# miha-stopar/Plonky3-mobile

Measured on AMD Instinct MI355X. Metric: fib_air proofs/sec, higher is better.
Workload: dtype u32 (BabyBear Montgomery, 31-bit modular)

## Files before the change

### plonky3-mobile_amd/csrc/mmcs.hip

```cpp
#include <algorithm>

#include "common.h"
#include "mmcs.h"
#include "poseidon2.hip.h"
#include "poseidon2_coop.hip.h"
#include "poseidon2_f64.hip.h"
#include "poseidon2_q4.hip.h"
#include "keccak.hip.h"

namespace p3 {

constexpr int MAX_CLASS_MATS = 16;

struct RowSet {
    const uint32_t* ptr[MAX_CLASS_MATS];
    uint32_t width[MAX_CLASS_MATS];
    uint32_t stride[MAX_CLASS_MATS];
    uint32_t count;
    uint32_t total;
};

__device__ __forceinline__ void load_digest(const uint32_t* p, uint32_t* out8) {
    const uint4* q = reinterpret_cast<const uint4*>(p);
    uint4 a = q[0], b = q[1];
    out8[0] = a.x; out8[1] = a.y; out8[2] = a.z; out8[3] = a.w;
    out8[4] = b.x; out8[5] = b.y; out8[6] = b.z; out8[7] = b.w;
}
__device__ __forceinline__ void store_digest(uint32_t* p, const uint32_t* s) {
    uint4* q = reinterpret_cast<uint4*>(p);
    q[0] = make_uint4(s[0], s[1], s[2], s[3]);
    q[1] = make_uint4(s[4], s[5], s[6], s[7]);
}

__device__ __forceinline__ void sponge_row(const RowSet& rs, uint64_t r, uint32_t (&s)[16]) {
#pragma unroll
    for (int i = 0; i < 16; i++) s[i] = 0;
    if (rs.count == 1) {
        const uint32_t* row = rs.ptr[0] + r * rs.stride[0];
        const uint32_t w = rs.width[0];
        for (uint32_t k = 0; k < w; k += 8) {
#pragma unroll
            for (int i = 0; i < 8; i++)
                if (k + i < w) s[i] = row[k + i];
            p2::permute(s);
        }
        return;
    }
    uint32_t m = 0, off = 0;
    for (uint32_t k = 0; k < rs.total; k += 8) {
#pragma unroll
        for (int i = 0; i < 8; i++) {
            if (k + i < rs.total) {
                while (off >= rs.width[m]) { m++; off = 0; }
                s[i] = rs.ptr[m][r * rs.stride[m] + off];
                off++;
            }
        }
        p2::permute(s);
    }
// ... 26 lines not shown
    }
    store_digest(next + i * 8, s);
}

__global__ void __launch_bounds__(256) tree_top_kernel(uint32_t* layer0, uint32_t n0) {
    P3_LATENCY_BOUND_KERNEL();
    extern __shared__ __attribute__((aligned(16))) uint32_t lds[];
    const uint32_t tid = threadIdx.x;
    for (uint32_t i = tid; i < n0 * 8; i += blockDim.x) lds[i] = layer0[i];
    __syncthreads();
    uint32_t* out = layer0 + (size_t)n0 * 8;
    for (uint32_t n = n0; n > 1; n >>= 1) {
        uint32_t half = n >> 1;
        uint32_t s[16];
        bool act = tid < half;
        if (act) {
#pragma unroll
            for (int k = 0; k < 16; k++) s[k] = lds[tid * 16 + k];
            p2::permute(s);
        }
        __syncthreads();
        if (act) {
#pragma unroll
            for (int k = 0; k < 8; k++) lds[tid * 8 + k] = s[k];
            store_digest(out + tid * 8, s);
        }
        __syncthreads();
        out += (size_t)half * 8;
    }
}


__global__ void __launch_bounds__(256) leaf_hash_f64_kernel(const uint32_t* mat, uint32_t width, uint64_t n_rows, uint32_t* digests) {
    if (gridDim.x <= 512u) P3_LATENCY_BOUND_KERNEL();
    uint64_t r = (uint64_t)blockIdx.x * blockDim.x + threadIdx.x;
    if (r >= n_rows) return;
    double s[16];
#pragma unroll
    for (int i = 0; i < 16; i++) s[i] = 0.0;
    const uint32_t* row = mat + r * width;
    for (uint32_t k = 0; k < width; k += 8) {
#pragma unroll
        for (int i = 0; i < 8; i++)
            if (k + i < width) s[i] = p2f::load_elem(row[k + i]);
        p2f::permute(s);
        if (k + 8 < width) {
#pragma unroll
            for (int i = 0; i < 16; i++) s[i] = p2f::reduce(s[i]);
        }
    }
    uint32_t d[8];
    const p2f::MagicRegs smk = p2f::magic_regs();
#pragma unroll
    for (int i = 0; i < 8; i++) d[i] = p2f::store_elem(s[i], smk);
    store_digest(digests + r * 8, d);
}
__global__ void __launch_bounds__(256) compress_layer_q4_kernel(const uint32_t* prev, uint32_t* next, uint64_t n_out, uint32_t prio) {
    if (prio) P3_LATENCY_BOUND_KERNEL();
    const uint32_t q = threadIdx.x & 3u;
    const uint64_t i = ((uint64_t)blockIdx.x * blockDim.x + threadIdx.x) >> 2;
    const bool act = i < n_out;
    const p2q::LaneConsts lc = p2q::lane_consts(q);
    double s[4] = {0.0, 0.0, 0.0, 0.0};
    if (act) {
        const uint4 w = *reinterpret_cast<const uint4*>(prev + i * 16 + 4 * q);
        s[0] = p2f::load_elem(w.x); s[1] = p2f::load_elem(w.y); s[2] = p2f::load_elem(w.z); s[3] = p2f::load_elem(w.w);
    }
    p2q::permute(s, lc, q == 0);
    if (act && q < 2) {
        const p2f::MagicRegs smk = p2f::magic_regs();
        *reinterpret_cast<uint4*>(next + i * 8 + 4 * q) =
            make_uint4(p2f::store_elem(s[0], smk), p2f::store_elem(s[1], smk), p2f::store_elem(s[2], smk), p2f::store_elem(s[3], smk));
    }
}
__global__ void __launch_bounds__(256) leaf_hash_q4_kernel(const uint32_t* mat, uint32_t width, uint64_t n_rows, uint32_t* digests, uint32_t prio) {
    if (prio) P3_LATENCY_BOUND_KERNEL();
    const uint32_t q = threadIdx.x & 3u;
    const uint64_t r = ((uint64_t)blockIdx.x * blockDim.x + threadIdx.x) >> 2;
    const bool act = r < n_rows;
    const p2q::LaneConsts lc = p2q::lane_consts(q);
    double s[4] = {0.0, 0.0, 0.0, 0.0};
    const uint32_t* row = mat + (act ? r : 0) * width;
    for (uint32_t k = 0; k < width; k += 8) {
        if (act && q < 2) {
#pragma unroll
            for (uint32_t i = 0; i < 4; i++)
                if (k + 4 * q + i < width) s[i] = p2f::load_elem(row[k + 4 * q + i]);
        }
        p2q::permute(s, lc, q == 0);
        if (k + 8 < width) {
#pragma unroll
            for (int i = 0; i < 4; i++) s[i] = p2f::reduce(s[i]);
        }
    }
    if (act && q < 2) {
        const p2f::MagicRegs smk = p2f::magic_regs();
        *reinterpret_cast<uint4*>(digests + r * 8 + 4 * q) =
            make_uint4(p2f::store_elem(s[0], smk), p2f::store_elem(s[1], smk), p2f::store_elem(s[2], smk), p2f::store_elem(s[3], smk));
    }
}
constexpr uint32_t LEAF_WIDE_CHUNK = 32, LEAF_WIDE_STRIDE = 36;
__global__ void __launch_bounds__(256) leaf_hash_f64_wide_kernel(const uint32_t* mat, uint32_t width, uint64_t n_rows, uint32_t* digests) {
    __shared__ __attribute__((aligned(16))) uint32_t tile[256 * LEAF_WIDE_STRIDE];
    const uint32_t tid = threadIdx.x, col = tid & 31u, rsub = tid >> 5;
    const uint64_t r0 = (uint64_t)blockIdx.x * 256u, r = r0 + tid;
    double s[16];
#pragma unroll
// ... 11 lines not shown
        __syncthreads();
#pragma unroll
        for (uint32_t i = 0; i < 32; i++) tile[(rsub + 8u * i) * LEAF_WIDE_STRIDE + col] = pre[i];
        __syncthreads();
        if (c0 + LEAF_WIDE_CHUNK < width) fetch(c0 + LEAF_WIDE_CHUNK);
        const uint4* mine = reinterpret_cast<const uint4*>(tile + tid * LEAF_WIDE_STRIDE);
#pragma unroll 1
        for (uint32_t k = 0; k < LEAF_WIDE_CHUNK && c0 + k < width; k += 8) {
            const uint4 a = mine[k / 4], b = mine[k / 4 + 1];
            const uint32_t w[8] = {a.x, a.y, a.z, a.w, b.x, b.y, b.z, b.w};
#pragma unroll
            for (int i = 0; i < 8; i++)
                if (c0 + k + i < width) s[i] = p2f::load_elem(w[i]);
            p2f::permute(s);
            if (c0 + k + 8 < width) {
#pragma unroll
                for (int i = 0; i < 16; i++) s[i] = p2f::reduce(s[i]);
            }
        }
    }
    if (r >= n_rows) return;
    uint32_t d[8];
    const p2f::MagicRegs smk = p2f::magic_regs();
#pragma unroll
    for (int i = 0; i < 8; i++) d[i] = p2f::store_elem(s[i], smk);
    store_digest(digests + r * 8, d);
}
__global__ void __launch_bounds__(256) leaf_hash_f64_rowset_kernel(RowSet rs, uint64_t n_rows, uint32_t* digests) {
    if (gridDim.x <= 512u) P3_LATENCY_BOUND_KERNEL();
    uint64_t r = (uint64_t)blockIdx.x * blockDim.x + threadIdx.x;
    if (r >= n_rows) return;
    double s[16];
#pragma unroll
    for (int i = 0; i < 16; i++) s[i] = 0.0;
    uint32_t m = 0, off = 0;
    for (uint32_t k = 0; k < rs.total; k += 8) {
#pragma unroll
        for (int i = 0; i < 8; i++) {
            if (k + i < rs.total) {
                while (off >= rs.width[m]) { m++; off = 0; }
                s[i] = p2f::load_elem(rs.ptr[m][r * rs.stride[m] + off]);
                off++;
            }
        }
        p2f::permute(s);
        if (k + 8 < rs.total) {
#pragma unroll
            for (int i = 0; i < 16; i++) s[i] = p2f::reduce(s[i]);
        }
    }
    uint32_t d[8];
    const p2f::MagicRegs smk = p2f::magic_regs();
#pragma unroll
    for (int i = 0; i < 8; i++) d[i] = p2f::store_elem(s[i], smk);
    store_digest(digests + r * 8, d);
}
__global__ void __launch_bounds__(256, 8) compress_layer_f64_kernel(const uint32_t* prev, uint32_t* next, uint64_t n_out) {
    if (gridDim.x <= 512u) P3_LATENCY_BOUND_KERNEL();
    uint64_t i = (uint64_t)blockIdx.x * blockDim.x + threadIdx.x;
    if (i >= n_out) return;
    uint32_t w[16];
    load_digest(prev + i * 16, w);
    load_digest(prev + i * 16 + 8, w + 8);
    double s[16];
#pragma unroll
    for (int k = 0; k < 16; k++) s[k] = p2f::load_elem(w[k]);
    p2f::permute(s);
    uint32_t d[8];
    const p2f::MagicRegs smk = p2f::magic_regs();
#pragma unroll
    for (int k = 0; k < 8; k++) d[k] = p2f::store_elem(s[k], smk);
    store_digest(next + i * 8, d);
}

__global__ void __launch_bounds__(256) compress_coop_kernel(const uint32_t* prev, uint32_t* next, uint32_t n_out) {
    P3_LATENCY_BOUND_KERNEL();
    const uint32_t lane16 = threadIdx.x & 15;
    const p2c::LaneConst lc = p2c::lane_constants(lane16);
    uint32_t i = (blockIdx.x * blockDim.x + threadIdx.x) >> 4;
    bool act = i < n_out;
    uint32_t v = act ? prev[(size_t)i * 16 + lane16] : 0u;
    v = p2c::permute(v, lc);
    if (act && lane16 < 8) next[(size_t)i * 8 + lane16] = v;
}
__global__ void __launch_bounds__(256) leaf_coop_kernel(const uint32_t* mat, uint32_t width, uint32_t n_rows, uint32_t* digests) {
    P3_LATENCY_BOUND_KERNEL();
    const uint32_t lane16 = threadIdx.x & 15;
    const p2c::LaneConst lc = p2c::lane_constants(lane16);
    uint32_t r = (blockIdx.x * blockDim.x + threadIdx.x) >> 4;
    bool act = r < n_rows;
    uint32_t v = 0;
    for (uint32_t k = 0; k < width; k += 8) {
        if (act && lane16 < 8 && k + lane16 < width) v = mat[(size_t)r * width + k + lane16];
        v = p2c::permute(v, lc);
    }
    if (act && lane16 < 8) digests[(size_t)r * 8 + lane16] = v;
}
__global__ void __launch_bounds__(1024) tree_levels_coop_kernel(uint32_t* layer_in, uint32_t n_in, uint32_t chunk, uint32_t levels,
                                                                uint32_t* root_copy) {
    P3_LATENCY_BOUND_KERNEL();
    __shared__ uint32_t lds[128 * 8];
    const uint32_t tid = threadIdx.x, lane16 = tid & 15, grp = tid >> 4;
    const p2c::LaneConst lc = p2c::lane_constants(lane16);
    const uint32_t* src = layer_in + (size_t)blockIdx.x * chunk * 8;
    for (uint32_t i = tid; i < chunk * 8; i += blockDim.x) lds[i] = src[i];
    __syncthreads();
    uint32_t* out = layer_in + (size_t)n_in * 8;
// ... 571 lines not shown
    constexpr uint32_t Q4_PRIO = 1;
    const uint64_t KCOOP_IN = profile == PROFILE_LATENCY ? (1ull << 12) : (1ull << 10);
    constexpr uint32_t KCOOP_CHUNK_LOG = 4;
    constexpr uint64_t KLANE_CHUNK = 1ull << 7;
    if (kind == HASH_KECCAK) {
        RowSet rs0 = make_rowset(*t, maxh);
        if (rs0.count == 1 && rs0.width[0] >= 68 && rs0.stride[0] == rs0.width[0])
            hipLaunchKernelGGL(keccak_leaf_wide_kernel, dim3((uint32_t)((maxh + 255) / 256)), dim3(256), 0, stream, rs0.ptr[0], rs0.width[0], maxh,
                               t->layers);
        else if (!launch_keccak_leaf_salted(stream, rs0, maxh, t->layers))
            hipLaunchKernelGGL(keccak_leaf_kernel, dim3((uint32_t)((maxh + 255) / 256)), dim3(256), 0, stream, rs0, maxh, t->layers);
        P3_HIP(hipGetLastError());
        for (size_t l = 1; l < t->layer_len.size(); l++) {
            uint64_t len = t->layer_len[l];
            RowSet rs = make_rowset(*t, len);
            if (len < COOP_MAX && !rs.count) {
                const uint64_t n_in = t->layer_len[l - 1];
                const bool coop = n_in <= KCOOP_IN;
                uint32_t levels = 0;
                while (levels < (coop ? KCOOP_CHUNK_LOG : 11u) && l + levels < t->layer_len.size() && !has_height(*t, t->layer_len[l + levels])) levels++;
                if (!coop) while (levels > 1 && (n_in >> levels) < KCOOP_IN) levels--;
                const uint32_t chunk = (uint32_t)std::min<uint64_t>(n_in, coop ? 1ull << KCOOP_CHUNK_LOG : KLANE_CHUNK);
                while ((1u << levels) > chunk) levels--;
                if (coop)
                    hipLaunchKernelGGL(keccak_tree_levels_coop_kernel, dim3((uint32_t)(n_in / chunk)), dim3(std::max<uint32_t>(64, chunk * 32)), 0,
                                       stream, t->layers + t->layer_off[l - 1], (uint32_t)n_in, chunk, levels, root_copy);
                else
                    hipLaunchKernelGGL(keccak_tree_levels_kernel, dim3((uint32_t)(n_in / chunk)), dim3(std::max<uint32_t>(64, chunk / 2)),
                                       (size_t)chunk * 32, stream, t->layers + t->layer_off[l - 1], (uint32_t)n_in, chunk, levels, root_copy);
                P3_HIP(hipGetLastError());
                if (t->layer_len[l + levels - 1] == 1) t->root_copied = root_copy != nullptr;
                l += levels - 1;
                continue;
            }
            hipLaunchKernelGGL(keccak_compress_kernel, dim3((uint32_t)((len + 255) / 256)), dim3(256), 0, stream,
                               t->layers + t->layer_off[l - 1], t->layers + t->layer_off[l], len, rs, rs.count > 0 ? 1u : 0u);
            P3_HIP(hipGetLastError());
        }
        *out = t.release();
        return OK;
    }
    {
        RowSet rs = make_rowset(*t, maxh);
        const bool dense1 = rs.count == 1 && rs.stride[0] == rs.width[0];
        if (dense1 && maxh < COOP_MAX && maxh * 16 <= 0x7fffffffull) {
            hipLaunchKernelGGL(leaf_coop_kernel, dim3((uint32_t)((maxh * 16 + 255) / 256)), dim3(256), 0, stream, rs.ptr[0],
                               rs.width[0], (uint32_t)maxh, t->layers);
        } else if (dense1 && maxh <= Q4_MAX && rs.width[0] <= 64 && (reinterpret_cast<uintptr_t>(t->layers) & 15u) == 0) {
            hipLaunchKernelGGL(leaf_hash_q4_kernel, dim3((uint32_t)((maxh * 4 + 255) / 256)), dim3(256), 0, stream, rs.ptr[0], rs.width[0], maxh,
                               t->layers, Q4_PRIO);
        } else if (dense1 && rs.width[0] >= 64) {
            hipLaunchKernelGGL(leaf_hash_f64_wide_kernel, dim3((uint32_t)((maxh + 255) / 256)), dim3(256), 0, stream, rs.ptr[0],
                               rs.width[0], maxh, t->layers);
        } else if (dense1) {
            hipLaunchKernelGGL(leaf_hash_f64_kernel, dim3((uint32_t)((maxh + 255) / 256)), dim3(256), 0, stream, rs.ptr[0],
                               rs.width[0], maxh, t->layers);
        } else if ((maxh >= COOP_MAX || (rs.count == 1 && !dense1))) {
            hipLaunchKernelGGL(leaf_hash_f64_rowset_kernel, dim3((uint32_t)((maxh + 255) / 256)), dim3(256), 0, stream, rs, maxh, t->layers);
        } else {
            hipLaunchKernelGGL(leaf_hash_kernel, dim3((uint32_t)((maxh + 255) / 256)), dim3(256), 0, stream, rs, maxh, t->layers);
        }
        P3_HIP(hipGetLastError());
    }
    for (size_t l = 1; l < t->layer_len.size();) {
        uint64_t len = t->layer_len[l];
        RowSet rs = make_rowset(*t, len);
        bool inject = rs.count > 0;
        if (!inject && len < COOP_MAX) {
            uint32_t levels = 0;
            while (levels < COOP_CHUNK_LOG && l + levels < t->layer_len.size() && !has_height(*t, t->layer_len[l + levels])) levels++;
            uint64_t n_in = t->layer_len[l - 1];
            uint32_t chunk = (uint32_t)std::min<uint64_t>(n_in, 1ull << COOP_CHUNK_LOG);
            while ((1u << levels) > chunk) levels--;
            uint32_t blocks = (uint32_t)(n_in / chunk);
            uint32_t threads = std::max<uint32_t>(64, chunk * 8);
            bool makes_root = t->layer_len[l + levels - 1] == 1;
            hipLaunchKernelGGL(tree_levels_coop_kernel, dim3(blocks), dim3(threads), 0, stream, t->layers + t->layer_off[l - 1],
                               (uint32_t)n_in, chunk, levels, makes_root ? root_copy : nullptr);
            P3_HIP(hipGetLastError());
            if (makes_root) t->root_copied = root_copy != nullptr;
            l += levels;
            continue;
        }
        if (!inject && len <= Q4_MAX) {
            hipLaunchKernelGGL(compress_layer_q4_kernel, dim3((uint32_t)((len * 4 + 255) / 256)), dim3(256), 0, stream,
                               t->layers + t->layer_off[l - 1], t->layers + t->layer_off[l], len, Q4_PRIO);
        } else if (!inject) {
            hipLaunchKernelGGL(compress_layer_f64_kernel, dim3((uint32_t)((len + 255) / 256)), dim3(256), 0, stream,
                               t->layers + t->layer_off[l - 1], t->layers + t->layer_off[l], len);
        } else {
            hipLaunchKernelGGL(compress_layer_kernel, dim3((uint32_t)((len + 255) / 256)), dim3(256), 0, stream,
                               t->layers + t->layer_off[l - 1], t->layers + t->layer_off[l], len, rs, inject ? 1u : 0u);
        }
        P3_HIP(hipGetLastError());
        l++;
    }
    *out = t.release();
    return OK;
}

int mmcs_root(hipStream_t stream, const Tree& t, uint32_t root_out[8]) {
    P3_HIP(hipMemcpyAsync(root_out, t.layers + t.layer_off.back(), 32, hipMemcpyDeviceToHost, stream));
    P3_HIP(hipStreamSynchronize(stream));
    return OK;
}

// ... 50 lines not shown
```

### plonky3-mobile_amd/csrc/prover.hip

```cpp
#include <chrono>
#include <cstddef>
#include <deque>
#include <memory>
#include <cstring>

#include "bb31.hip.h"
#include "challenger.h"
#include "common.h"
#include "keccak.hip.h"
#include "mmcs.h"
#include "poseidon2.hip.h"
#include "poseidon2_f64.hip.h"
#include "prover.h"
#include "rng.h"
#include "rng_dev.hip.h"
#include "transcript.hip.h"

namespace p3 {

using bb::Ext;

__device__ __forceinline__ uint32_t tl(const TwoLevelTable& t, uint32_t e) {
    return bb::mul(t.lo[e & ((1u << t.T) - 1u)], t.hi[e >> t.T]);
}
__device__ __forceinline__ uint32_t brev(uint32_t v, uint32_t bits) { return bits ? (__brev(v) >> (32 - bits)) : 0u; }

__device__ __forceinline__ Ext ld_ext(const uint32_t* p) {
    uint4 v = *reinterpret_cast<const uint4*>(p);
    return Ext{{v.x, v.y, v.z, v.w}};
}
__device__ __forceinline__ void st_ext(uint32_t* p, const Ext& e) {
    *reinterpret_cast<uint4*>(p) = make_uint4(e.c[0], e.c[1], e.c[2], e.c[3]);
}

constexpr int SEL_CHUNK = 8;
__global__ void selectors_kernel(TwoLevelTable roots, uint32_t n, uint32_t gen, uint32_t ginv, uint32_t zh, uint2* sel) {
    uint32_t t = blockIdx.x * blockDim.x + threadIdx.x;
    uint32_t i0 = t * SEL_CHUNK;
    if (i0 >= n) return;
    uint32_t v[2 * SEL_CHUNK], pre[2 * SEL_CHUNK];
    uint32_t acc = bb::ONE;
#pragma unroll
    for (int k = 0; k < SEL_CHUNK; k++) {
        uint32_t x = bb::mul(gen, tl(roots, (i0 + k) & (n - 1)));
        v[2 * k] = bb::sub(x, bb::ONE);
        v[2 * k + 1] = bb::sub(x, ginv);
    }
#pragma unroll
    for (int k = 0; k < 2 * SEL_CHUNK; k++) { pre[k] = acc; acc = bb::mul(acc, v[k]); }
    uint32_t inv = bb::mul(bb::inv(acc), zh);
#pragma unroll
    for (int k = 2 * SEL_CHUNK - 1; k >= 0; k--) {
        uint32_t r = bb::mul(inv, pre[k]);
        inv = bb::mul(inv, v[k]);
        v[k] = r;
    }
#pragma unroll
    for (int k = 0; k < SEL_CHUNK; k++)
        if (i0 + k < n) sel[i0 + k] = make_uint2(v[2 * k], v[2 * k + 1]);
}

struct QuotArgs {
    const uint2* lde;
    const uint2* sel;
    uint32_t* out;
// ... 129 lines not shown
    uint32_t* ro;
    const DevState* ds;
    uint32_t big;
};
__global__ void __launch_bounds__(256) reduced_openings_kernel(ReducedArgs a) {
    uint32_t j = blockIdx.x * blockDim.x + threadIdx.x;
    if (j >= a.big) return;
    const DevState* __restrict__ ds = a.ds;
    uint2 t = a.lde_t[j];
    uint4 q = a.lde_q[j];
    Ext u, w;
#pragma unroll
    for (int c = 0; c < 4; c++) {
        u.c[c] = bb::add(bb::add(bb::dot2(ds->alp[4].c[c], q.x, ds->alp[5].c[c], q.y), bb::dot2(ds->alp[6].c[c], q.z, ds->alp[7].c[c], q.w)),
                         bb::mul(ds->alp[1].c[c], t.y));
        w.c[c] = bb::dot2(ds->alp[2].c[c], t.x, ds->alp[3].c[c], t.y);
    }
    u.c[0] = bb::add(u.c[0], t.x);
    Ext e0 = ld_ext(a.d0 + 4 * (size_t)j), e1 = ld_ext(a.d1 + 4 * (size_t)j);
    Ext r = bb::add(bb::mul(bb::sub(ds->y02, u), e0), bb::mul(bb::sub(ds->y1, w), e1));
    st_ext(a.ro + 4 * (size_t)j, r);
}

__global__ void __launch_bounds__(256) fri_fold_kernel(TwoLevelTable inv_roots , const uint32_t* in,
                                                       uint32_t* out, uint32_t half, uint32_t log_half,
                                                       const DevState* __restrict__ ds, uint32_t round, uint32_t one_half) {
    if (gridDim.x <= 512u) P3_LATENCY_BOUND_KERNEL();
    uint32_t i = blockIdx.x * blockDim.x + threadIdx.x;
    if (i >= half) return;
    const Ext half_beta = ds->half_beta[round];
    Ext lo = ld_ext(in + 8 * (size_t)i), hi = ld_ext(in + 8 * (size_t)i + 4);
    uint32_t p = tl(inv_roots, brev(i, log_half));
    Ext s = bb::scale(bb::add(lo, hi), one_half);
    Ext d = bb::mul(bb::scale(half_beta, p), bb::sub(lo, hi));
    st_ext(out + 4 * (size_t)i, bb::add(s, d));
}

__global__ void __launch_bounds__(256) fri_fold_rollin_kernel(TwoLevelTable inv_roots , const uint32_t* in,
                                                              const uint32_t* __restrict__ ro, uint32_t* out, uint32_t half,
                                                              uint32_t log_half, const DevState* __restrict__ ds, uint32_t round,
                                                              uint32_t one_half) {
    if (gridDim.x <= 512u) P3_LATENCY_BOUND_KERNEL();
    uint32_t i = blockIdx.x * blockDim.x + threadIdx.x;
    if (i >= half) return;
    const Ext half_beta = ds->half_beta[round];
    const Ext beta2 = bb::sqr(bb::add(half_beta, half_beta));
    Ext lo = ld_ext(in + 8 * (size_t)i), hi = ld_ext(in + 8 * (size_t)i + 4), e = ld_ext(ro + 4 * (size_t)i);
    uint32_t p = tl(inv_roots, brev(i, log_half));
    Ext s = bb::scale(bb::add(lo, hi), one_half);
    Ext d = bb::mul(bb::scale(half_beta, p), bb::sub(lo, hi));
    st_ext(out + 4 * (size_t)i, bb::add(bb::add(s, d), bb::mul(beta2, e)));
}

__global__ void __launch_bounds__(256, 8) grind_kernel(DevState* ds, uint32_t mask, uint32_t base) {
    uint32_t w = base + blockIdx.x * blockDim.x + threadIdx.x;
    if (w >= bb::P) return;
    if (base + blockIdx.x * blockDim.x > *(volatile uint32_t*)&ds->grind_result) return;
    const uint32_t pos = ds->n_in;
    double s[16];
#pragma unroll
    for (int i = 0; i < 16; i++) s[i] = p2f::load_elem((i < 8 && (uint32_t)i < pos) ? ds->inb[i & 7] : ds->st[i]);
#pragma unroll
    for (int i = 0; i < 8; i++) s[i] = (i == (int)pos) ? (double)w : s[i];
    p2f::permute(s);
    if ((bb::from_monty(p2f::store_elem(s[7])) & mask) == 0) atomicMin(&ds->grind_result, w);
}

__global__ void __launch_bounds__(256) grind_keccak_kernel(DevState* ds, uint32_t mask, uint32_t base) {
    uint32_t w = base + blockIdx.x * blockDim.x + threadIdx.x;
    if (w >= bb::P) return;
    if (base + blockIdx.x * blockDim.x > *(volatile uint32_t*)&ds->grind_result) return;
    const KeccakGrindArgs& a = ds->kgrind;
    const uint32_t wm = bb::to_monty(w);
    uint64_t st[25];
#pragma unroll
    for (int i = 0; i < 25; i++) st[i] = a.state[i];
    for (uint32_t blk = 0; blk < a.n_blocks; blk++) {
#pragma unroll
        for (int i = 0; i < 17; i++) {
            uint64_t lane = a.block[blk][i];
            const int32_t rel = (int32_t)(a.wpos) - (int32_t)(blk * 136 + i * 8);
            if (rel > -4 && rel < 8) {
                const uint64_t v = (uint64_t)wm;
                lane ^= rel >= 0 ? (v << (8 * rel)) : (v >> (8 * -rel));
            }
            st[i] ^= lane;
        }
        if (blk + 1 == a.n_blocks) kk::permute_digest(st);
        else kk::permute(st);
    }
    bool ok = false;
#pragma unroll
    for (int t = 0; t < 8; t++) {
        const uint64_t lane = st[3 - t / 2];
        const uint32_t hi_or_lo = (t & 1) ? (uint32_t)lane : (uint32_t)(lane >> 32);
        const uint32_t v = __builtin_bswap32(hi_or_lo) & 0x7fffffffu;
        if (v < bb::P) { ok = (v & mask) == 0; break; }
    }
    if (ok) atomicMin(&ds->grind_result, w);
}

constexpr uint32_t QTREE_MAX_MATS = 8;
struct QTree {
    const uint32_t* mat[QTREE_MAX_MATS];
    uint32_t width[QTREE_MAX_MATS];
    uint32_t stride[QTREE_MAX_MATS];
    uint32_t n_mats;
    const uint32_t* layers;
    uint32_t log_height, shift, slot_off;
    uint32_t mshift[QTREE_MAX_MATS];
};
__global__ void query_gather_kernel(const QTree* trees, const uint32_t* indices, uint32_t slot_words, uint32_t* out) {
    P3_LATENCY_BOUND_KERNEL();
    const QTree& t = trees[blockIdx.y];
    const uint64_t index = (indices[blockIdx.x] >> t.shift) & ((1ull << t.log_height) - 1ull);
    uint32_t* dst = out + (size_t)blockIdx.x * slot_words + t.slot_off;
    uint32_t off = 0;
    for (uint32_t m = 0; m < t.n_mats; m++) {
// ... 174 lines not shown
            uint32_t res = 0;
            if (base + wave_first < half) {
                const uint32_t v = (row < half && lane16 < 8) ? vbuf[cur][row * 8 + lane16] : 0u;
                res = p2c::permute(v, lc);
            }
            if (row < half && lane16 < 8) { dig[0][row * 8 + lane16] = res; lay[row * 8 + lane16] = res; }
        }
        __syncthreads();
        uint32_t d = 0;
        size_t off = (size_t)half * 8;
        for (uint32_t n = half; n > 1; n >>= 1) {
            const uint32_t m = n >> 1;
            uint32_t res = 0;
            if (wave_first < m) {
                const uint32_t v = grp < m ? dig[d][grp * 16 + lane16] : 0u;
                res = p2c::permute(v, lc);
            }
            if (grp < m && lane16 < 8) { dig[d ^ 1][grp * 8 + lane16] = res; lay[off + grp * 8 + lane16] = res; }
            __syncthreads();
            d ^= 1;
            off += (size_t)m * 8;
        }
        const uint32_t round = a.r0 + k;
        if (tid < 8) a.ts.ps[a.ts.lay.froots + 8 * round + tid] = dig[d][tid];
        if (tid < 64) {
            for (uint32_t i = 0; i < 8; i++) ch.observe(dig[d][i]);
            const Ext beta = ch.sample_ext();
            if (tid == 0) { hb = bb::scale(beta, a.one_half); a.ts.ds->half_beta[round] = hb; }
        }
        __syncthreads();
        if (tid < half) {
            const Ext half_beta = hb;
            const Ext lo = ld_ext(&vbuf[cur][8 * tid]), hi = ld_ext(&vbuf[cur][8 * tid + 4]);
            const uint32_t p = tl(a.inv_roots[k], brev(tid, log_half));
            const Ext r = bb::add(bb::scale(bb::add(lo, hi), a.one_half), bb::mul(bb::scale(half_beta, p), bb::sub(lo, hi)));
            st_ext(&vbuf[cur ^ 1][4 * tid], r);
            st_ext(a.vec + a.vec_off[k + 1] + 4 * (size_t)tid, r);
        }
        __syncthreads();
        cur ^= 1;
    }
    if (tid < 64) ch.end();
}

__global__ void __launch_bounds__(64) ts_final_kernel(TsArgs a, uint32_t fpl, uint32_t pow_mask) {
    P3_LATENCY_BOUND_KERNEL();
    __shared__ KState ks;
    DevChal ch;
    ch.begin(a.kind, a.ds, &ks, false);
    for (uint32_t i = 0; i < 4 * fpl; i++) ch.observe(a.ps[a.lay.fpoly + i]);
    ch.end();
    if (threadIdx.x == 0) {
        a.ds->grind_result = 0xffffffffu;
        if (a.kind == HASH_KECCAK) {
            KeccakGrindArgs& g = a.ds->kgrind;
            for (int i = 0; i < 25; i++) g.state[i] = ks.st[i];
            uint8_t tmpl[272];
            for (int i = 0; i < 272; i++) tmpl[i] = 0;
            const uint32_t tail = ks.blen;
            for (uint32_t i = 0; i < tail; i++) tmpl[i] = ks.blk[i];
            const uint32_t end = tail + 4;
            g.n_blocks = end < 136 ? 1 : 2;
            tmpl[end] ^= 0x01;
            tmpl[g.n_blocks * 136 - 1] ^= 0x80;
            for (int b = 0; b < 2; b++)
                for (int i = 0; i < 17; i++) {
                    uint64_t w = 0;
                    for (int j = 0; j < 8; j++) w |= (uint64_t)tmpl[b * 136 + 8 * i + j] << (8 * j);
                    g.block[b][i] = w;
                }
            g.wpos = tail;
            g.mask = pow_mask;
            g.base = 0;
        }
    }
}
__global__ void __launch_bounds__(64) ts_queries_kernel(TsArgs a, uint32_t nq, uint32_t log_big, uint32_t pow_bits, uint32_t* qidx) {
    P3_LATENCY_BOUND_KERNEL();
    __shared__ KState ks;
    const uint32_t found = a.ds->grind_result;
    if (found == 0xffffffffu) {
        if (threadIdx.x == 0) { a.ds->status = ST_GRIND_MISS; a.ps[a.lay.status] = ST_GRIND_MISS; }
        for (uint32_t q = threadIdx.x; q < nq; q += 64) qidx[q] = 0;
        return;
    }
    DevChal ch;
    ch.begin(a.kind, a.ds, &ks, false);
    const uint32_t witness = bb::to_monty(found);
    ch.observe(witness);
    const uint32_t zero_bits = ch.sample_bits(pow_bits);
    if (threadIdx.x == 0) {
        a.ps[a.lay.witness] = witness;
        a.ps[a.lay.status] = zero_bits == 0 ? 0u : 2u;
        a.ds->status = 0;
    }
    for (uint32_t q = 0; q < nq; q++) {
        const uint32_t idx = ch.sample_bits(log_big);
        if (threadIdx.x == 0) { qidx[q] = idx; a.ps[a.lay.qidx + q] = idx; }
    }
    ch.end();
}

static void put_u32(std::vector<uint8_t>& b, uint32_t v) {
    size_t o = b.size();
    b.resize(o + 4);
    memcpy(b.data() + o, &v, 4);
// ... 108 lines not shown
    int commit(size_t n, const uint32_t* const* mats, const size_t* widths, uint32_t* const* salts, size_t height, uint32_t* layers,
               uint32_t root_slot, size_t mat_stride = 0, hipStream_t on = nullptr) {
        hipStream_t cs = on ? on : stream;
        const uint32_t* mp[QTREE_MAX_MATS]; size_t hh[QTREE_MAX_MATS], ww[QTREE_MAX_MATS], ss[QTREE_MAX_MATS];
        size_t k = 0;
        for (size_t i = 0; i < n; i++, k++) {
            mp[k] = mats[i]; hh[k] = height; ww[k] = widths[i]; ss[k] = mat_stride ? mat_stride : widths[i];
            if (salt_words) { k++; mp[k] = salts[i]; hh[k] = height; ww[k] = ss[k] = salt_words; }
        }
        Tree* tp = nullptr;
        int r = mmcs_commit(cs, mp, hh, ww, k, &tp, layers, pstage + root_slot, hash, ss, profile);
        if (r) return r;
        std::unique_ptr<Tree> t(tp);
        if (!t->root_copied) P3_HIP(hipMemcpyAsync(pstage + root_slot, t->layers + t->layer_off.back(), 32, hipMemcpyDeviceToDevice, cs));
        return OK;
    }
    int fri_rounds(Context& cx, const TsArgs& ts, uint32_t r_end, const uint32_t* const* rollin = nullptr) {
        const uint32_t one_half = bb::inv(bb::to_monty(2));
        const size_t row = 8;
        int rc;
        for (uint32_t r = 0; r < r_end; r++) {
            const uint32_t log_half = log_big - 1 - r, half = 1u << log_half;
            uint32_t* vec = fri_vec + fri_vec_off[r];
            uint32_t* salts = salt_words ? fri_salts + fri_salt_off[r] : nullptr;
            if ((rc = commit(1, &vec, &row, &salts, half, fri_layers + fri_layer_off[r], lay.froots + 8 * r))) return rc;
            hipLaunchKernelGGL(ts_fri_round_kernel, dim3(1), dim3(64), 0, stream, ts, r, one_half);
            P3_HIP(hipGetLastError());
            TwoLevelTable inv_roots;
            if ((rc = cx.get_root_table(stream, log_half + 1, true, &inv_roots))) return rc;
            if (rollin && rollin[r])
                hipLaunchKernelGGL(fri_fold_rollin_kernel, dim3((half + 255) / 256), dim3(256), 0, stream, inv_roots, vec, rollin[r],
                                   fri_vec + fri_vec_off[r + 1], half, log_half, ts.ds, r, one_half);
            else
                hipLaunchKernelGGL(fri_fold_kernel, dim3((half + 255) / 256), dim3(256), 0, stream, inv_roots, vec, fri_vec + fri_vec_off[r + 1],
                                   half, log_half, ts.ds, r, one_half);
            P3_HIP(hipGetLastError());
        }
        return OK;
    }
    int fri_final(Context& cx, const TsArgs& ts) {
        const uint32_t fpl = 1u << fp.log_final_poly_len;
        int rc;
        if ((rc = bit_reverse_rows(stream, fri_vec + fri_vec_off[n_rounds], fp_ev, fpl, 4))) return rc;
        if ((rc = ntt_dft(cx, stream, fp_ev, pstage + lay.fpoly, fpl, 4, true))) return rc;
        hipLaunchKernelGGL(ts_final_kernel, dim3(1), dim3(64), 0, stream, ts, fpl, pow_mask());
        P3_HIP(hipGetLastError());
        return OK;
    }

    uint32_t pow_mask() const { return (1u << fp.proof_of_work_bits) - 1u; }
    uint32_t grind_range(uint32_t first_log) const {
        return 1u << std::min<uint32_t>(std::max<uint32_t>(first_log ? first_log : fp.proof_of_work_bits + 4, 8), 24);
    }
    int grind(const TsArgs& ts, uint64_t base, uint32_t count) {
        if (hash == HASH_KECCAK) hipLaunchKernelGGL(grind_keccak_kernel, dim3(count / 256), dim3(256), 0, stream, ts.ds, pow_mask(), (uint32_t)base);
        else hipLaunchKernelGGL(grind_kernel, dim3(count / 256), dim3(256), 0, stream, ts.ds, pow_mask(), (uint32_t)base);
        P3_HIP(hipGetLastError());
        return OK;
    }
    int grind_start(const TsArgs& ts) {
        const uint32_t first_log = grind_first_log(), batch = grind_range(first_log);
        const uint32_t head = first_log ? batch : std::min<uint32_t>(batch, 1u << std::max<uint32_t>(fp.proof_of_work_bits + 1, 8));
        int rc;
        if ((rc = grind(ts, 0, head))) return rc;
        if (batch > head && (rc = grind(ts, head, batch - head))) return rc;
        return OK;
    }
    int queries(const TsArgs& ts, uint32_t* host, size_t words) {
        const uint32_t nq = fp.num_queries;
        hipLaunchKernelGGL(ts_queries_kernel, dim3(1), dim3(64), 0, stream, ts, nq, log_big, fp.proof_of_work_bits, qidx);
        P3_HIP(hipGetLastError());
        if (nq) {
            hipLaunchKernelGGL(query_gather_kernel, dim3(nq, (uint32_t)trees.size()), dim3(64), 0, stream, qtrees, qidx, (uint32_t)slot_words,
                               pstage + lay.slots);
            P3_HIP(hipGetLastError());
        }
        P3_HIP(hipMemcpyAsync(host, pstage, words * 4, hipMemcpyDeviceToHost, stream));
        return OK;
    }
    int continue_grind(const TsArgs& ts, uint32_t* host, size_t words) {
        uint32_t batch = grind_range(grind_first_log()), found = 0xffffffffu;
        int rc;
        for (uint64_t base = batch; base < bb::P && found == 0xffffffffu; base += batch) {
            batch = std::min<uint32_t>(batch * 4, 1u << 24);
            if ((rc = grind(ts, base, batch))) return rc;
            P3_HIP(hipMemcpyAsync(&found, &ts.ds->grind_result, 4, hipMemcpyDeviceToHost, stream));
            P3_HIP(hipStreamSynchronize(stream));
        }
        if (found == 0xffffffffu) return fail(ERR_INTERNAL, "grind: no proof-of-work witness found");
        if ((rc = queries(ts, host, words))) return rc;
        P3_HIP(hipStreamSynchronize(stream));
        return OK;
    }

    void put_fri(std::vector<uint8_t>& pf, const uint32_t* hp) const {
        const StageLayout& L = lay;
        const uint32_t nq = fp.num_queries, fpl = 1u << fp.log_final_poly_len, n_inputs = (uint32_t)trees.size() - n_rounds;
        put_u32(pf, n_rounds); put_words(pf, hp + L.froots, (size_t)n_rounds * 8);
        put_u32(pf, nq);
        for (uint32_t q = 0; q < nq; q++) {
            const uint32_t* slot = hp + L.slots + (size_t)q * slot_words;
            put_u32(pf, n_inputs);
            for (uint32_t i = 0; i < n_inputs; i++) {
                const QTree& t = trees[i];
                put_opening(pf, slot, salt_words ? t.n_mats / 2 : t.n_mats, t.width, salt_words, t.log_height);
            }
            put_u32(pf, n_rounds);
            for (uint32_t r = 0; r < n_rounds; r++) {
                const uint32_t lh = log_big - 1 - r, idx = hp[L.qidx + q] >> r;
                put_words(pf, slot + 4 * ((idx ^ 1) & 1), 4);
                if (salt_words) { put_u32(pf, salt_words); put_words(pf, slot + 8, salt_words); }
                put_u32(pf, lh); put_words(pf, slot + 8 + salt_words, (size_t)lh * 8);
                slot += 8 + salt_words + (size_t)lh * 8;
            }
        }
        put_u32(pf, fpl);
        put_words(pf, hp + L.fpoly, (size_t)fpl * 4);
        put_u32(pf, hp[L.witness]);
    }
};

constexpr int N_STAGE_EVENTS = 7;

struct FibProver::Impl : ProverCore {
    uint32_t log_n = 0;
    uint32_t *trace = nullptr, *lde_t = nullptr, *qflat = nullptr, *lde_q = nullptr, *d0 = nullptr, *d1 = nullptr;
    uint32_t *layers_t = nullptr, *layers_q = nullptr, *partials = nullptr;
    DevState* ds = nullptr;
    uint32_t* host_stage[2] = {nullptr, nullptr};
    hipEvent_t done[2] = {nullptr, nullptr};
    struct Pending {
        uint64_t a, b; int slot; std::chrono::steady_clock::time_point t_start, t_enq; uint64_t seq;
        const uint32_t* trace;
        TsPis pis;
    };
    std::deque<Pending> pending;
    uint64_t next_seq = 1, arena_owner = 0;
    hipEvent_t ev[2][N_STAGE_EVENTS] = {{nullptr}, {nullptr}};
// ... 286 lines not shown
```

### plonky3-mobile_amd/csrc/transcript.hip.h

```cpp
#pragma once
#include "bb31.hip.h"
#include "keccak.hip.h"
#include "mmcs.h"
#include "poseidon2_coop.hip.h"

namespace p3 {

struct DenConsts {
    uint32_t z0, z1, z2, z3, k0, k1, c1, z2w, z3w;
};
BB_HD DenConsts den_consts(const bb::Ext& z) {
    DenConsts k{};
    k.z0 = z.c[0]; k.z1 = z.c[1]; k.z2 = z.c[2]; k.z3 = z.c[3];
    const uint32_t W = bb::W_MONTY;
    uint32_t b0 = bb::add(bb::sqr(z.c[1]), bb::mul(W, bb::sqr(z.c[3]))), b1 = bb::dbl(bb::mul(z.c[1], z.c[3]));
    uint32_t c0 = bb::mul(W, b1);
    k.c1 = b0;
    k.k0 = bb::sub(bb::mul(W, bb::sqr(z.c[2])), c0);
    k.k1 = bb::dbl(z.c[2]);
    k.z2w = bb::mul(W, z.c[2]);
    k.z3w = bb::mul(W, z.c[3]);
    return k;
}

struct KeccakGrindArgs {
    uint64_t state[25];
    uint64_t block[2][17];
    uint32_t n_blocks, wpos;
    uint32_t mask, base;
};

constexpr uint32_t MAX_FRI_ROUNDS = 32;
constexpr uint32_t ST_GRIND_MISS = 1u;

struct KState {
    uint64_t st[25];
    uint32_t blen, n_obuf;
    alignas(8) uint8_t blk[136];
    alignas(8) uint8_t obuf[32];
};
static_assert(sizeof(KState) % 8 == 0, "KState is copied as 64-bit words");

struct DevState {
    uint32_t st[16], inb[8], outb[8], n_in, n_out;
    KState kc;
    uint32_t pis[4];
    bb::Ext apow[5];
    bb::Ext zeta, zeta_next;
    DenConsts k0, k1;
    bb::Ext alp[8], y02, y1;
    bb::Ext half_beta[MAX_FRI_ROUNDS];
    uint32_t grind_result;
    uint32_t status;
    KeccakGrindArgs kgrind;
};

__device__ __forceinline__ void lds_wave_sync() {
    __builtin_amdgcn_fence(__ATOMIC_SEQ_CST, "wavefront");
    __builtin_amdgcn_wave_barrier();
}
__device__ __noinline__ void k_absorb_block(KState* k) {
    const uint32_t lane = threadIdx.x & 63u, idx = kk::coop_index();
    lds_wave_sync();
    uint64_t a = idx < 25u ? k->st[idx] : 0ull;
    if (idx < 17u) {
        uint64_t w = 0;
#pragma unroll
        for (int b = 0; b < 8; b++) w |= (uint64_t)k->blk[8 * idx + b] << (8 * b);
        a ^= w;
    }
    a = kk::f_coop(a);
    if (idx < 25u) k->st[idx] = a;
    if (lane == 0) k->blen = 0;
    lds_wave_sync();
}
__device__ __forceinline__ void k_observe_byte(KState* k, uint8_t b) {
    const uint32_t bl = k->blen;
    if ((threadIdx.x & 63u) == 0) { k->n_obuf = 0; k->blk[bl] = b; k->blen = bl + 1; }
    lds_wave_sync();
    if (bl + 1 == 136) k_absorb_block(k);
}
__device__ __forceinline__ void k_observe_word(KState* k, uint32_t v) {
    const uint32_t bl = k->blen;
    if (bl & 3u) {
        for (int i = 0; i < 4; i++) k_observe_byte(k, (uint8_t)(v >> (8 * i)));
        return;
    }
    if ((threadIdx.x & 63u) == 0) { k->n_obuf = 0; *reinterpret_cast<uint32_t*>(k->blk + bl) = v; k->blen = bl + 4; }
    lds_wave_sync();
    if (bl + 4 == 136) k_absorb_block(k);
}
__device__ __noinline__ void k_flush(KState* k) {
    const uint32_t lane = threadIdx.x & 63u, n = k->blen;
    for (uint32_t i = n + lane; i < 136; i += 64) k->blk[i] = 0;
    lds_wave_sync();
    if (lane == 0) { k->blk[n] ^= 0x01; k->blk[135] ^= 0x80; }
    k_absorb_block(k);
    uint8_t byte = 0;
    if (lane < 32u) byte = (uint8_t)(k->st[lane >> 3] >> (8 * (lane & 7u)));
    lds_wave_sync();
    if (lane < 25u) k->st[lane] = 0;
    if (lane < 32u) { k->obuf[lane] = byte; k->blk[lane] = byte; }
    if (lane == 0) { k->blen = 32; k->n_obuf = 32; }
    lds_wave_sync();
}
__device__ __noinline__ uint32_t k_sample(KState* k) {
    for (;;) {
// ... 97 lines not shown
```

Before: 572.9.

## Specialize narrow-row leaf hashing and make Poseidon2 grinding use persistent ticketed walkers

Adds a leaf hash kernel for dense matrices with one to eight columns. It folds the known-zero capacity into a specialised first external linear layer and computes only the eight output lanes in the last layer. The Poseidon2 grind kernel becomes a persistent grid of up to 128 blocks that pull 256-nonce ranges from an atomic ticket counter. Each block stops early once a smaller solution is found, and the head/tail split launch for Poseidon2 is dropped. The changes also add a cheaper store_elem variant, and they add an extra memset per grind batch plus atomic ticket contention.

```diff
diff --git a/plonky3-mobile_amd/csrc/mmcs.hip b/plonky3-mobile_amd/csrc/mmcs.hip
--- a/plonky3-mobile_amd/csrc/mmcs.hip
+++ b/plonky3-mobile_amd/csrc/mmcs.hip
@@ -5,6 +5,7 @@
 #include "poseidon2.hip.h"
 #include "poseidon2_coop.hip.h"
 #include "poseidon2_f64.hip.h"
+#include "poseidon2_f64_leaf.hip.h"
 #include "poseidon2_q4.hip.h"
 #include "keccak.hip.h"
 
@@ -137,7 +138,24 @@
     uint32_t d[8];
     const p2f::MagicRegs smk = p2f::magic_regs();
 #pragma unroll
-    for (int i = 0; i < 8; i++) d[i] = p2f::store_elem(s[i], smk);
+    for (int i = 0; i < 8; i++) d[i] = p2f::store_elem_i(s[i], smk);
+    store_digest(digests + r * 8, d);
+}
+__global__ void __launch_bounds__(256, 8) leaf_hash_f64_block_kernel(const uint32_t* mat, uint32_t width, uint64_t n_rows, uint32_t* digests) {
+    if (gridDim.x <= 512u) P3_LATENCY_BOUND_KERNEL();
+    uint64_t r = (uint64_t)blockIdx.x * blockDim.x + threadIdx.x;
+    if (r >= n_rows) return;
+    double s[16];
+    const uint32_t* row = mat + r * width;
+#pragma unroll
+    for (int i = 0; i < 8; i++) s[i] = (uint32_t)i < width ? p2f::load_elem(row[i]) : 0.0;
+    p2f::external_linear_first_n(s, width);
+    const p2f::MagicRegs mk = p2f::magic_regs();
+    p2f::permute_inner(s, mk);
+    p2f::external_linear_last8(s);
+    uint32_t d[8];
+#pragma unroll
+    for (int i = 0; i < 8; i++) d[i] = p2f::store_elem_i(s[i], mk);
     store_digest(digests + r * 8, d);
 }
 __global__ void __launch_bounds__(256) compress_layer_q4_kernel(const uint32_t* prev, uint32_t* next, uint64_t n_out, uint32_t prio) {
@@ -255,7 +273,7 @@
     uint32_t d[8];
     const p2f::MagicRegs smk = p2f::magic_regs();
 #pragma unroll
-    for (int i = 0; i < 8; i++) d[i] = p2f::store_elem(s[i], smk);
+    for (int i = 0; i < 8; i++) d[i] = p2f::store_elem_i(s[i], smk);
     store_digest(digests + r * 8, d);
 }
 __global__ void __launch_bounds__(256, 8) compress_layer_f64_kernel(const uint32_t* prev, uint32_t* next, uint64_t n_out) {
@@ -933,6 +951,9 @@
         } else if (dense1 && rs.width[0] >= 64) {
             hipLaunchKernelGGL(leaf_hash_f64_wide_kernel, dim3((uint32_t)((maxh + 255) / 256)), dim3(256), 0, stream, rs.ptr[0],
                                rs.width[0], maxh, t->layers);
+        } else if (dense1 && rs.width[0] >= 1 && rs.width[0] <= 8) {
+            hipLaunchKernelGGL(leaf_hash_f64_block_kernel, dim3((uint32_t)((maxh + 255) / 256)), dim3(256), 0, stream, rs.ptr[0],
+                               rs.width[0], maxh, t->layers);
         } else if (dense1) {
             hipLaunchKernelGGL(leaf_hash_f64_kernel, dim3((uint32_t)((maxh + 255) / 256)), dim3(256), 0, stream, rs.ptr[0],
                                rs.width[0], maxh, t->layers);
diff --git a/plonky3-mobile_amd/csrc/poseidon2_f64_leaf.hip.h b/plonky3-mobile_amd/csrc/poseidon2_f64_leaf.hip.h
--- /dev/null
+++ b/plonky3-mobile_amd/csrc/poseidon2_f64_leaf.hip.h
@@ -0,0 +1,95 @@
+#pragma once
+#include "poseidon2_f64.hip.h"
+
+namespace p2f {
+
+template <int W>
+__device__ __forceinline__ void mat4_lead(double& a, double& b, double& c, double& d) {
+    static_assert(W >= 1 && W <= 4, "one to four leading elements");
+    if constexpr (W == 4) {
+        mat4(a, b, c, d);
+    } else if constexpr (W == 3) {
+        const double t01 = a + b, t0123 = t01 + c, t01123 = t0123 + b;
+        const double nd = __fma_rn(a, 2.0, t0123), nb = __fma_rn(c, 2.0, t01123);
+        const double na = t01123 + t01, nc = t0123 + c;
+        a = na; b = nb; c = nc; d = nd;
+    } else if constexpr (W == 2) {
+        const double t01 = a + b, t01123 = t01 + b;
+        const double nd = __fma_rn(a, 2.0, t01), na = t01123 + t01;
+        a = na; b = t01123; c = t01; d = nd;
+    } else {
+        const double na = a + a, nd = __fma_rn(a, 2.0, a);
+        b = a; c = a; d = nd; a = na;
+    }
+}
+template <int W>
+__device__ __forceinline__ void external_linear_first(double (&s)[16]) {
+    static_assert(W >= 1 && W <= 8, "the rate is eight words");
+    if constexpr (W <= 4) {
+        mat4_lead<W>(s[0], s[1], s[2], s[3]);
+#pragma unroll
+        for (int i = 0; i < 4; i++) {
+            s[4 + i] = s[i]; s[8 + i] = s[i]; s[12 + i] = s[i];
+            s[i] = s[i] + s[i];
+        }
+    } else {
+        mat4(s[0], s[1], s[2], s[3]);
+        mat4_lead<W - 4>(s[4], s[5], s[6], s[7]);
+#pragma unroll
+        for (int i = 0; i < 4; i++) {
+            const double t = s[i] + s[4 + i];
+            s[8 + i] = t; s[12 + i] = t;
+            s[i] += t; s[4 + i] += t;
+        }
+    }
+}
+__device__ __forceinline__ void external_linear_first_n(double (&s)[16], uint32_t w) {
+    switch (w) {
+    case 1: external_linear_first<1>(s); break;
+    case 2: external_linear_first<2>(s); break;
+    case 3: external_linear_first<3>(s); break;
+    case 4: external_linear_first<4>(s); break;
+    case 5: external_linear_first<5>(s); break;
+    case 6: external_linear_first<6>(s); break;
+    case 7: external_linear_first<7>(s); break;
+    default: external_linear_first<8>(s); break;
+    }
+}
+__device__ __forceinline__ void external_linear_last8(double (&s)[16]) {
+#pragma unroll
+    for (int i = 0; i < 16; i += 4) mat4(s[i], s[i + 1], s[i + 2], s[i + 3]);
+#pragma unroll
+    for (int k = 0; k < 4; k++) {
+        const double t = (s[k] + s[k + 4]) + (s[k + 8] + s[k + 12]);
+        s[k] += t; s[k + 4] += t;
+    }
+}
+
+__device__ __forceinline__ void permute_inner(double (&s)[16], const MagicRegs& mk) {
+    const double npm1 = d_c.neg_pm1, pinv = d_c.pinv;
+    _Pragma("clang loop unroll(disable)")
+    for (int r = 0; r < 4; r++) {
+#pragma unroll
+        for (int i = 0; i < 16; i++) s[i] = sbox7(s[i] + d_c.ext[r][i], mk, npm1, pinv);
+        external_linear(s);
+    }
+    internal_rounds(s, mk);
+    _Pragma("clang loop unroll(disable)")
+    for (int r = 4; r < 7; r++) {
+#pragma unroll
+        for (int i = 0; i < 16; i++) s[i] = sbox7(s[i] + d_c.ext[r][i], mk, npm1, pinv);
+        external_linear(s);
+    }
+#pragma unroll
+    for (int i = 0; i < 16; i++) s[i] = sbox7(s[i] + d_c.ext[7][i], mk, npm1, pinv);
+}
+
+__device__ __forceinline__ uint32_t store_elem_i(double v, const MagicRegs& k) {
+    const double qb = __fma_rn(v, R_MOD_P_OVER_P, k.m);
+    const double c = __fma_rn(qb, d_c.neg_pm1, k.mp);
+    const double t = __fma_rn(R_MOD_P, v, c);
+    const uint32_t w = (uint32_t)__double2loint(t) - (uint32_t)__double2loint(qb);
+    return min(w, w + bb::P);
+}
+
+}
diff --git a/plonky3-mobile_amd/csrc/prover.hip b/plonky3-mobile_amd/csrc/prover.hip
--- a/plonky3-mobile_amd/csrc/prover.hip
+++ b/plonky3-mobile_amd/csrc/prover.hip
@@ -11,6 +11,7 @@
 #include "mmcs.h"
 #include "poseidon2.hip.h"
 #include "poseidon2_f64.hip.h"
+#include "poseidon2_f64_leaf.hip.h"
 #include "prover.h"
 #include "rng.h"
 #include "rng_dev.hip.h"
@@ -246,18 +247,33 @@
     st_ext(out + 4 * (size_t)i, bb::add(bb::add(s, d), bb::mul(beta2, e)));
 }
 
-__global__ void __launch_bounds__(256, 8) grind_kernel(DevState* ds, uint32_t mask, uint32_t base) {
-    uint32_t w = base + blockIdx.x * blockDim.x + threadIdx.x;
-    if (w >= bb::P) return;
-    if (base + blockIdx.x * blockDim.x > *(volatile uint32_t*)&ds->grind_result) return;
-    const uint32_t pos = ds->n_in;
-    double s[16];
-#pragma unroll
-    for (int i = 0; i < 16; i++) s[i] = p2f::load_elem((i < 8 && (uint32_t)i < pos) ? ds->inb[i & 7] : ds->st[i]);
-#pragma unroll
-    for (int i = 0; i < 8; i++) s[i] = (i == (int)pos) ? (double)w : s[i];
-    p2f::permute(s);
-    if ((bb::from_monty(p2f::store_elem(s[7])) & mask) == 0) atomicMin(&ds->grind_result, w);
+constexpr uint32_t GRIND_WALKERS = 128;
+__global__ void __launch_bounds__(256, 8) grind_kernel(DevState* ds, uint32_t mask, uint32_t base, uint32_t n_ranges) {
+    __shared__ uint32_t drawn;
+    const p2f::MagicRegs mk = p2f::magic_regs();
+    for (;;) {
+        if (threadIdx.x == 0) {
+            uint32_t t = atomicAdd(&ds->grind_ticket, 1u);
+            if (t >= n_ranges || base + t * 256u > *(volatile uint32_t*)&ds->grind_result) t = 0xffffffffu;
+            drawn = t;
+        }
+        __syncthreads();
+        const uint32_t t = drawn;
+        __syncthreads();
+        if (t == 0xffffffffu) return;
+        const uint32_t w = base + t * 256u + threadIdx.x;
+        if (w >= bb::P) continue;
+        const uint32_t pos = ds->n_in;
+        double s[16];
+#pragma unroll
+        for (int i = 0; i < 16; i++) s[i] = p2f::load_elem((i < 8 && (uint32_t)i < pos) ? ds->inb[i & 7] : ds->st[i]);
+#pragma unroll
+        for (int i = 0; i < 8; i++) s[i] = (i == (int)pos) ? (double)w : s[i];
+        p2f::external_linear(s);
+        p2f::permute_inner(s, mk);
+        p2f::external_linear_last8(s);
+        if ((bb::from_monty(p2f::store_elem_i(s[7], mk)) & mask) == 0) atomicMin(&ds->grind_result, w);
+    }
 }
 
 __global__ void __launch_bounds__(256) grind_keccak_kernel(DevState* ds, uint32_t mask, uint32_t base) {
@@ -538,6 +554,7 @@
     ch.end();
     if (threadIdx.x == 0) {
         a.ds->grind_result = 0xffffffffu;
+        a.ds->grind_ticket = 0;
         if (a.kind == HASH_KECCAK) {
             KeccakGrindArgs& g = a.ds->kgrind;
             for (int i = 0; i < 25; i++) g.state[i] = ks.st[i];
@@ -752,18 +769,24 @@
     uint32_t grind_range(uint32_t first_log) const {
         return 1u << std::min<uint32_t>(std::max<uint32_t>(first_log ? first_log : fp.proof_of_work_bits + 4, 8), 24);
     }
-    int grind(const TsArgs& ts, uint64_t base, uint32_t count) {
-        if (hash == HASH_KECCAK) hipLaunchKernelGGL(grind_keccak_kernel, dim3(count / 256), dim3(256), 0, stream, ts.ds, pow_mask(), (uint32_t)base);
-        else hipLaunchKernelGGL(grind_kernel, dim3(count / 256), dim3(256), 0, stream, ts.ds, pow_mask(), (uint32_t)base);
+    int grind(const TsArgs& ts, uint64_t base, uint32_t count, bool first) {
+        if (hash == HASH_KECCAK) {
+            hipLaunchKernelGGL(grind_keccak_kernel, dim3(count / 256), dim3(256), 0, stream, ts.ds, pow_mask(), (uint32_t)base);
+        } else {
+            if (!first) P3_HIP(hipMemsetAsync(&ts.ds->grind_ticket, 0, 4, stream));
+            const uint32_t n_ranges = count / 256;
+            hipLaunchKernelGGL(grind_kernel, dim3(std::min(n_ranges, GRIND_WALKERS)), dim3(256), 0, stream, ts.ds, pow_mask(), (uint32_t)base, n_ranges);
+        }
         P3_HIP(hipGetLastError());
         return OK;
     }
     int grind_start(const TsArgs& ts) {
         const uint32_t first_log = grind_first_log(), batch = grind_range(first_log);
+        if (hash != HASH_KECCAK) return grind(ts, 0, batch, true);
         const uint32_t head = first_log ? batch : std::min<uint32_t>(batch, 1u << std::max<uint32_t>(fp.proof_of_work_bits + 1, 8));
         int rc;
-        if ((rc = grind(ts, 0, head))) return rc;
-        if (batch > head && (rc = grind(ts, head, batch - head))) return rc;
+        if ((rc = grind(ts, 0, head, true))) return rc;
+        if (batch > head && (rc = grind(ts, head, batch - head, false))) return rc;
         return OK;
     }
     int queries(const TsArgs& ts, uint32_t* host, size_t words) {
@@ -783,7 +806,7 @@
         int rc;
         for (uint64_t base = batch; base < bb::P && found == 0xffffffffu; base += batch) {
             batch = std::min<uint32_t>(batch * 4, 1u << 24);
-            if ((rc = grind(ts, base, batch))) return rc;
+            if ((rc = grind(ts, base, batch, false))) return rc;
             P3_HIP(hipMemcpyAsync(&found, &ts.ds->grind_result, 4, hipMemcpyDeviceToHost, stream));
             P3_HIP(hipStreamSynchronize(stream));
         }
diff --git a/plonky3-mobile_amd/csrc/transcript.hip.h b/plonky3-mobile_amd/csrc/transcript.hip.h
--- a/plonky3-mobile_amd/csrc/transcript.hip.h
+++ b/plonky3-mobile_amd/csrc/transcript.hip.h
@@ -53,6 +53,7 @@
     uint32_t grind_result;
     uint32_t status;
     KeccakGrindArgs kgrind;
+    uint32_t grind_ticket;
 };
 
 __device__ __forceinline__ void lds_wave_sync() {
```

After: 543.4. 5.1% lower.
